# bioXiaoheng/BallerMixPlus

Measured on AMD Instinct MI355X. Metric: CLR windows/sec (B2 scan, n=100), higher is better.
Workload: dtype f64; 1 GPU; BASELINE config 4: synthetic whole genome, 39999999 SNPs over 22 chromosomes (GRCh37 proportions), n=100, default 31x10x51 (A,x,alpha) grid, B2 scan, every SNP a test site; site arrays of all chromosomes resident on every GPU, test sites dealt to the GPUs in blocks of 4096; grid_points=15810, library_build=8afc0fca11e6a83d

## Files before the change

### ballermixplus_amd/csrc/bmxscan.hip

```cpp
#include <hip/hip_runtime.h>
#include <stdint.h>
#include <stdio.h>
#include <stdlib.h>
#include <string.h>

#include <dlfcn.h>
#include <errno.h>
#include <rccl/rccl.h>

#include <algorithm>
#include <atomic>
#include <mutex>
#include <type_traits>
#include <string>
#include <thread>
#include <unordered_set>
#include <vector>

#include "../../include/bmxscan.h"
#include "bmx_math.h"

namespace {

thread_local std::string g_err;
// ... 1137 lines not shown
                    acc[i + 1] *= fma(Fs[i + 1], v0, 1.0);
                }
                __builtin_amdgcn_wave_barrier();
            } else {
                for (int b = L_int; b < R_int; b += SP) generic_pass(b, +1, R_int, staged);
            }
            PROF_MARK(0);
            int b = bulk_zone(R_int, +1, tL, t0);
            if (b != ZONE_DONE) { CNT(12, 1); while (!generic_pass(b, +1, N, false)) { b += SP; CNT(12, 1); } }
            PROF_MARK(7);
            b = bulk_zone(L_int - 1, -1, t0, tL);
            if (b != ZONE_DONE) { CNT(12, 1); while (!generic_pass(b, -1, -1, false)) { b -= SP; CNT(12, 1); } }
            PROF_MARK(7);

            renorm_all();
#pragma unroll
            for (int j = 0; j < J; ++j) {
                const int ec = min(max(E[j], -131071), 131071) + 131072;
                const int eb = bestK[j] >> 13;
                const bool better = (ec > eb) || (ec == eb && acc[j] > bestM[j]);
                if (better && p < P.npairs) {
                    bestM[j] = acc[j];
                    bestK[j] = (ec << 13) | iA;
                }
            }
        }
#pragma unroll
        for (int j = 0; j < J; ++j) {
            const int biA = bestK[j] & 8191;
            int bE = bestK[j] >> 13;
            double bM = bestM[j];
            int bL = biA == 8191 ? 0x7fffffff : biA * P.npairs + p;
            for (int off = 32; off > 0; off >>= 1) {
                const int oE = __shfl_xor(bE, off);
                const double oM = __shfl_xor(bM, off);
                const int oL = __shfl_xor(bL, off);
                if (oE > bE || (oE == bE && (oM > bM || (oM == bM && oL < bL)))) { bE = oE; bM = oM; bL = oL; }
            }
            if (lane == 0 && j < nvalid) {
                const size_t o = (size_t)slice * P.M + (tb + j);
                P.part_T[o] = bM;
                P.part_lin[o] = bL;
                P.part_ns[o] = bE;
            }
        }
    }
#ifdef BMX_PROFILE
    if (lane == 0 && P.prof)
        for (int k = 0; k < 12; ++k) atomicAdd(P.prof + k, (unsigned long long)prof_[k]);
#endif
#ifdef BMX_COUNT
    if (lane == 0 && P.prof)
        for (int k = 0; k < 16; ++k) atomicAdd(P.prof + 16 + k, cnt_[k]);
#endif
}

#ifndef BMX_P_ORDER
#define BMX_P_ORDER 12
#endif
constexpr int P_ORDER = BMX_P_ORDER;
constexpr int P_COPIES = 4;
static_assert(P_ORDER == 8 || P_ORDER == 12 || P_ORDER == 16, "far-field order of the prepared kernels: 8, 12 or 16");
static_assert(P_COPIES * P_ORDER <= WAVE, "slot-0 copies must fit one wave-wide read");
constexpr double P_EPS = P_ORDER == 16 ? 0.25 : P_ORDER == 12 ? 0.15 : 0.05;
constexpr int P_FAR_CAP = P_ORDER == 16 ? 2048 : P_ORDER == 12 ? 3584 : 8192;
#if BMX_P_ORDER == 16
__device__ constexpr double P_W[16] = {0.9999999999999954, 0.4999999999999791, 0.3333333333368442, 0.250000000008901, 0.19999999921757028,
                                       0.1666666652123534, 0.14285722101681053, 0.1250001188192722, 0.11110698172974029, 0.09999456222768308,
                                       0.09103227543438049, 0.08347880124963403, 0.07484961178075682, 0.06918273076087589, 0.08475562956871537,
                                       0.08074032343426385};
__device__ constexpr double P_D[14] = {9.539, 6.739, 5.071, 3.966, 3.181, 2.594, 2.14, 1.778, 1.483, 1.237, 1.03, 0.853, 0.7, 0.566};
#elif BMX_P_ORDER == 12
__device__ constexpr double P_W[12] = {0.9999999999999661, 0.49999999999988076, 0.3333333333754503, 0.25000000008463336, 0.19999998506452038,
                                       0.1666666441614055, 0.14285940976674, 0.1250028457483109, 0.11094429253027539, 0.09981580095968261,
                                       0.09676290425438011, 0.08920395582674094};
__device__ constexpr double P_D[10] = {9.029, 6.228, 4.56, 3.455, 2.67, 2.084, 1.629, 1.267, 0.972, 0.726};
#else
__device__ constexpr double P_W[8] = {0.9999999999998467, 0.4999999999996164, 0.3333333341509627, 0.25000000122701976,
                                      0.19999882322703955, 0.16666529319200146, 0.1434841013671569, 0.12562715480255862};
__device__ constexpr double P_D[6] = {7.94, 5.13, 3.462, 2.357, 1.571, 0.985};
#endif
constexpr double P_RAG_D = P_ORDER == 16 ? 6.74 : P_ORDER == 12 ? 6.23 : 5.13;
constexpr int PREP_HDR = 3, PREP_GUARD = 8, PREP_MOM = 1 + P_ORDER / 2, PREP_RAG_GUARD = 1;
constexpr double SER_DMIN = P_ORDER > 8 ? P_D[P_ORDER > 8 ? 6 : 0] : 0.0;
constexpr int SER_CAP = 64;
constexpr int PREP_MAGIC = 0x5a0e0000;
constexpr int RING_UNITS = 256, RING_MIRROR = 32, AUX_UNITS = 32;
constexpr int PREP_ZONE_DONE = -0x7fffffff;
constexpr int PREP_THREADS = 256;
constexpr int PREP_THR_LDS_MAX = 4096;
constexpr int64_t SOLO_GAP = 10;

struct PrepParams {
    const double *genpos;
    RowArray row;
    int64_t N;
    int rows, rowmul;
    const double *A;
    int nA;
    const double *test_gen;
    const int64_t *win_lo, *win_hi, *center, *center_hi;
    int64_t M;
    double zcut;
    const double *rowthr;
    int thr_in_lds;
    const uint8_t *kmom;
    const int *row_of_slot;
    int mom_slots;
    int ser_cap;
    int64_t g_begin, g_end;
    int32_t *blob_units;
    const int64_t *blob_prefix;
    int64_t prefix_base;
    ScratchEnt *arena;
    int *status;
};

template <int J, bool FILL>
__global__ __launch_bounds__(PREP_THREADS) void prep_kernel(PrepParams P) {
    extern __shared__ __attribute__((aligned(16))) double lds_p[];
    const int lane = threadIdx.x & (WAVE - 1);
    const int wave = __builtin_amdgcn_readfirstlane((int)(threadIdx.x >> 6));
    const int nw = blockDim.x / WAVE;
    const int N = (int)P.N;
    const int thr_len = P.thr_in_lds ? ((P.rows + 1) & ~1) : 0;
    if (P.thr_in_lds) {
        for (int idx = threadIdx.x; idx < P.rows; idx += blockDim.x) lds_p[idx] = P.rowthr[idx];
        __syncthreads();
    }
    constexpr int MS = FILL ? P_ORDER : 1;
    const int mom_len = (P.mom_slots + P_COPIES - 1 + 3) * MS;
    double *mom_r = lds_p + thr_len + wave * (2 * mom_len + WAVE);
    double *mom_l = mom_r + mom_len;
    double *ragscr = mom_l + mom_len;
    ScratchEnt *ser_r = reinterpret_cast<ScratchEnt *>(lds_p + thr_len + nw * (2 * mom_len + WAVE)) + wave * (2 * SER_CAP);
    ScratchEnt *ser_l = ser_r + SER_CAP;
    for (int idx = lane; idx < 2 * mom_len; idx += WAVE) mom_r[idx] = 0.0;
    __builtin_amdgcn_wave_barrier();
    const int64_t grp = P.g_begin + (int64_t)blockIdx.x * nw + wave;
    if (grp >= P.g_end) return;
    auto thr_of = [&](int r) -> double {
        double v;
        if (P.thr_in_lds) v = lds_p[r]; else v = P.rowthr[r];
        return v;
    };
    auto rank = [&](unsigned long long m) {
        return (int)__builtin_amdgcn_mbcnt_hi((unsigned)(m >> 32), __builtin_amdgcn_mbcnt_lo((unsigned)m, 0u));
    };
    constexpr int BS = J >= 16 ? 4 : 8;

    const int64_t tb = grp * J;
    const int nvalid = (int)min((int64_t)J, P.M - tb);
    const int jl = lane % J;
    const int jj = min(jl, nvalid - 1);
    const double tj = P.test_gen[tb + jj];
    int lo_j = (int)max(P.win_lo[tb + jj], (int64_t)0);
    int hi_j = (int)min(P.win_hi[tb + jj], (int64_t)N - 1);
    if (jl >= nvalid) { lo_j = 1; hi_j = 0; }
    const double t0 = readlane_f64(tj, 0), tL = readlane_f64(tj, J - 1);
    const int c0 = (int)P.center[tb], cU = (int)P.center_hi[tb + nvalid - 1];
    int lo_max = 0, hi_min = N - 1;
#pragma unroll
    for (int j = 0; j < J; ++j) {
        const int a = __builtin_amdgcn_readlane(lo_j, j), b = __builtin_amdgcn_readlane(hi_j, j);
        if (j < nvalid) { lo_max = max(lo_max, a); hi_min = min(hi_min, b); }
    }
    int L_int = min(c0, hi_min + 1), R_int = max(cU, lo_max);
    if (hi_min < lo_max) { L_int = c0; R_int = c0; hi_min = -1; lo_max = N; }

    int wpos = 0;
    ScratchEnt *out = nullptr;
    if (FILL) out = P.arena + (P.blob_prefix[grp] - P.prefix_base);

    for (int iA = 0; iA < P.nA; ++iA) {
        const double A = P.A[iA];
        const int kmom = min((int)P.kmom[iA], P.mom_slots);
        auto zone_near = [&](int base, int dir, double tnear, double tfar, double *mom, ScratchEnt *ser, int &zbase_o, int &npp_o, int &nqp_o,
                             int &nfar_o, int &base_o, double &m1p_o, double &m2p_o, int &nragv_o, int &nrmax_o, int &rag_o, double &zr_o,
                             int &rr_o, int &nser_o) {
            const int zbase = wpos, nbase = zbase + PREP_HDR;
            int n_pair = 0, n_pair_pad = 0, n_quad = 0, nfar_tot = 0, pad_ro = 0, n_ser = 0;
            bool pair_open = true, seen = false;
            double m1p = 0.0, m2p = 0.0;
            auto close_pairs = [&]() {
                n_pair_pad = (n_pair + BS - 1) & ~(BS - 1);
                if (FILL && lane < n_pair_pad - n_pair) out[nbase + n_pair + lane] = ScratchEnt{0.0, pad_ro, 0};
                pair_open = false;
            };
            int i = base + dir * lane;
            double g_nx = P.genpos[min(max(i, 0), N - 1)];
            int r_nx = (int)P.row[min(max(i, 0), N - 1)];
            while (true) {
                const bool ok = dir > 0 ? (i <= hi_min) : (i >= lo_max);
                const double g = g_nx;
                const int rraw = r_nx;
                const int inx = i + dir * WAVE;
                g_nx = P.genpos[min(max(inx, 0), N - 1)];
                r_nx = (int)P.row[min(max(inx, 0), N - 1)];
                const bool bulk = ok && (A * fabs(g - tfar) <= P.zcut);
                const int cnt = __popcll(__ballot(bulk));
                if (cnt) {
                    const double zn = A * fabs(g - tnear);
                    const double th = thr_of(rraw);
                    const int slot = __double2loint(th) & 0xff;
                    const bool farx = bulk && zn >= th && nfar_tot + n_ser < P_FAR_CAP;
                    const bool moml = farx && slot < kmom;
                    const bool serx = farx && slot >= kmom && !(zn - th < SER_DMIN);
                    const unsigned long long ms_ = __ballot(serx);
                    const bool ser_ok = n_ser + __popcll(ms_) <= P.ser_cap;
                    const bool serl = ser_ok && serx;
                    const bool nearl = bulk && !moml && !serl;
                    const bool pairl = nearl && zn < LN2;
                    const unsigned long long mm = __ballot(moml), mp = __ballot(pairl), mq = __ballot(nearl && !pairl);
                    const int nfar = __popcll(mm);
                    if (!seen) { pad_ro = __builtin_amdgcn_readlane(rraw, 0) * P.rowmul; seen = true; }
                    double Ev = 0.0;
                    if (FILL) Ev = bulk ? exp_neg(zn) : 0.0;
                    if (nfar) {
                        if (moml) {
                            double *mr = mom + (slot ? slot + P_COPIES - 1 : (lane & (P_COPIES - 1))) * MS;
                            if (FILL) {
                                const double d = zn - th;
                                const double E2 = Ev * Ev;
                                if (slot == 0) { m1p += Ev; m2p += E2; }
                                else { atomicAdd(mr, Ev); atomicAdd(mr + 1, E2); }
                                double Ek = E2;
#pragma unroll
                                for (int k = 3; k <= P_ORDER; ++k) {
                                    if (!(d < P_D[k - 3])) break;
                                    Ek *= Ev;
                                    atomicAdd(mr + (k - 1), Ek);
                                }
                            } else {
                                mom[(slot ? slot + P_COPIES - 1 : 0) * MS] = 1.0;
                            }
                        }
                        nfar_tot += nfar;
                    }
                    if (ser_ok && ms_ != 0ull) {
                        if (FILL && serl) {
                            const double d = zn - th;
                            const int cls = !(d < P_D[0]) ? 2 : !(d < P_D[1]) ? 3 : !(d < P_D[3]) ? 5 : 8;
                            ser[n_ser + rank(ms_)] = ScratchEnt{Ev, rraw * P.rowmul, cls};
                        }
                        n_ser += __popcll(ms_);
                    }
                    if (pair_open) {
                        if (FILL && pairl) out[nbase + n_pair + rank(mp)] = ScratchEnt{Ev, rraw * P.rowmul, 0};
                        n_pair += __popcll(mp);
                        if (__ballot(bulk && !(zn < LN2)) != 0ull || cnt < WAVE) close_pairs();
                    }
                    if (!pair_open) {
                        if (FILL && nearl && !pairl) out[nbase + n_pair_pad + n_quad + rank(mq)] = ScratchEnt{Ev, rraw * P.rowmul, 0};
                        n_quad += __popcll(mq);
                    }
                }
                base += dir * cnt;
                if (cnt < WAVE) break;
                i = inx;
            }
            if (pair_open) close_pairs();
            const int n_quad_pad = (n_quad + 3) & ~3;
            if (FILL) {
                if (lane < n_quad_pad - n_quad) out[nbase + n_pair_pad + n_quad + lane] = ScratchEnt{0.0, pad_ro, 0};
                if (lane < PREP_GUARD) out[nbase + n_pair_pad + n_quad_pad + lane] = ScratchEnt{0.0, pad_ro, 0};
            }
            wpos = nbase + n_pair_pad + n_quad_pad + PREP_GUARD;

            int nrag_v = 0, nrmax = 0;
            int rag = 0;
            double zr = 0.0;
            int rr = 0;
            {
                const int ir = base + dir * lane;
                const bool inr = ir >= 0 && ir < N;
                const int ic = min(max(ir, 0), N - 1);
                const double g = P.genpos[ic];
                rr = (int)P.row[ic];
                bool okr = __ballot(inr && (dir > 0 ? g <= tnear : g >= tnear)) == 0ull &&
                           __ballot(dir > 0 ? lo_j > base : hi_j < base) == 0ull;
                if (okr) {
                    ragscr[lane] = g;
                    __builtin_amdgcn_wave_barrier();
                    const int cnt1 = min(max(dir > 0 ? hi_j - base + 1 : base - lo_j + 1, 0), WAVE);
                    int lo_n = 0, hi_n = WAVE;
#pragma unroll
                    for (int it = 0; it < 7; ++it) {
                        const int mid = min((lo_n + hi_n) >> 1, WAVE - 1);
                        const bool pm = A * fabs(ragscr[mid] - tj) <= P.zcut;
                        const bool act = lo_n < hi_n;
                        lo_n = act && pm ? mid + 1 : lo_n;
                        hi_n = act && !pm ? mid : hi_n;
                    }
                    nrag_v = min(cnt1, lo_n);
                    __builtin_amdgcn_wave_barrier();
                    const int nb = dir > 0 ? __shfl_up(nrag_v, 1) : __shfl_down(nrag_v, 1);
                    const bool edge = dir > 0 ? jl == 0 : jl == J - 1;
                    okr = __ballot(!edge && nb > nrag_v) == 0ull;
                    nrmax = __builtin_amdgcn_readlane(nrag_v, dir > 0 ? J - 1 : 0);
                }
                if (okr && nrmax > 0 && nrmax < WAVE) {
                    zr = A * fabs(g - tnear);
                    const bool far8 = lane >= nrmax || zr >= thr_of(rr) + SER_DMIN;
                    const bool far3 = lane >= nrmax || zr >= thr_of(rr) + P_RAG_D;
                    rag = __ballot(far8) == ~0ull ? (__ballot(far3) == ~0ull ? 1 : 3) : 0;
                }
            }
            if (rag) {
                if (FILL) {
                    if (lane < nrmax) out[wpos + lane] = ScratchEnt{exp_neg(zr), rr * P.rowmul, zr >= thr_of(rr) + P_RAG_D ? 0 : 1};
                    if (lane == nrmax) out[wpos + lane] = ScratchEnt{0.0, rr * P.rowmul, 0};
                }
                wpos += nrmax + PREP_RAG_GUARD;
            }
            zbase_o = zbase; npp_o = n_pair_pad; nqp_o = n_quad_pad; nfar_o = nfar_tot; base_o = base; m1p_o = m1p; m2p_o = m2p;
            nragv_o = nrag_v; nrmax_o = nrmax; rag_o = rag; zr_o = zr; rr_o = rr; nser_o = n_ser;
        };
        auto zone_far = [&](double *mom, const ScratchEnt *ser, int n_ser, int zbase, int n_pair_pad, int n_quad_pad, int nfar_tot, int base,
                            double m1p, double m2p, int nrag_v, int nrmax, int rag, double zr, int rr) {
            int n_occ = 0;
            if (nfar_tot) {
                __builtin_amdgcn_wave_barrier();
                {
                    double x = 0.0;
                    if (lane < P_COPIES * MS) {
                        x = mom[lane];
                        mom[lane] = 0.0;
                    }
                    if (FILL) {
                        double y1 = m1p, y2 = m2p;
#pragma unroll
                        for (int off = 1; off < WAVE; off <<= 1) {
                            y1 += __shfl_xor(y1, off);
                            y2 += __shfl_xor(y2, off);
                        }
                        x += lane == 0 ? y1 : lane == 1 ? y2 : 0.0;
// ... 385 lines not shown
        int E[J], bestK[J];
#pragma unroll
        for (int j = 0; j < J; ++j) {
            bestM[j] = BMX_FREXP ? 0.5 : 1.0;
            bestK[j] = ((131072 + (BMX_FREXP ? 1 : 0)) << 13) | 8191;
        }

        for (int iA = 0; iA < P.nA; ++iA) {
            const double A = P.A[iA];
            int bits = 0;
#pragma unroll
            for (int j = 0; j < J; ++j) { acc[j] = 1.0; E[j] = 0; }
            auto renorm_all = [&]() {
#pragma unroll
                for (int j = 0; j < J; ++j) {
                    if (BMX_FREXP) renorm_fx(acc[j], E[j]); else renorm(acc[j], E[j]);
                }
                bits = 0;
            };
            auto spend = [&](int nbits) {
                if (bits + nbits > 1000) renorm_all();
                bits += nbits;
            };
            const int span_generic = max(P.span_hi, 54);

            auto apply_pass = [&](double alpha, int rowoff, unsigned long long m_in, double *buf) {
                buf[lane] = alpha;
                __builtin_amdgcn_wave_barrier();
                double Rpre[SP];
                if (!USE_LDS) {
#pragma unroll
                    for (int s = 0; s < SP; ++s) Rpre[s] = loadR(__builtin_amdgcn_readlane(rowoff, s * J));
                }
#pragma unroll
                for (int s = 0; s < SP; ++s) {
                    if (((m_in >> (s * J)) & ((1ull << J) - 1ull)) == 0ull) continue;
                    const double R = USE_LDS ? loadR(__builtin_amdgcn_readlane(rowoff, s * J)) : Rpre[s];
                    const double2 *a2 = reinterpret_cast<const double2 *>(buf + s * J);
#pragma unroll
                    for (int j = 0; j < J; j += 2) {
                        const double2 a = a2[j >> 1];
                        acc[j] *= fma(a.x, R, 1.0);
                        acc[j + 1] *= fma(a.y, R, 1.0);
                    }
                }
                __builtin_amdgcn_wave_barrier();
            };
            auto generic_core = [&](int i, bool inr, double g, int rowoff, int dir) -> bool {
                const bool inwin = inr && i >= lo_j && i <= hi_j;
                const double z = A * fabs(g - tj);
                const bool in = inwin && (z <= P.zcut) && (g != tj);
                const bool fin = lo_j > hi_j ||
                                 (dir > 0 ? (!inr || i > hi_j || (i >= lo_j && g > tj && z > P.zcut))
                                          : (!inr || i < lo_j || (i <= hi_j && g < tj && z > P.zcut)));
                const unsigned long long m_in = __ballot(in);
                if (m_in != 0ull) {
                    const double alpha = in ? exp_neg(z) : 0.0;
                    spend(SP * (__ballot(in && z < 0.6931471805599453) == 0ull ? max(P.span_hi, 2) : span_generic));
                    apply_pass(alpha, rowoff, m_in, scr_d);
                }
                return __ballot(fin) == ~0ull;
            };
            auto generic_pass = [&](int b, int dir, int lim, bool from_lds) -> bool {
                const int i = b + dir * sl;
                const bool inr = dir > 0 ? (i < lim) : (i > lim);
                double g = 0.0;
                int rowoff = 0;
                if (from_lds) {
                    if (inr) { g = mid_g[i - L_int]; rowoff = mid_ro[i - L_int]; }
                } else {
                    if (inr) { g = P.genpos[i]; rowoff = (int)P.row[i] * rowmul; }
                }
                return generic_core(i, inr, g, rowoff, dir);
            };

            auto zone_near = [&](auto dirk, double tnear, double &fv_o, int &nocc_o, int &nfar_o, int &nrmax_o, int &rag_o, int &nser_o,
                                 FargVec &farg) -> int {
                constexpr int dirc = decltype(dirk)::value;
                int nragv_o = 0;
                nocc_o = 0; nfar_o = 0; nrmax_o = 0; rag_o = 0; nser_o = 0;
                fv_o = 0.0;
                if (bad) return PREP_ZONE_DONE;
                double F[J];
                {
                    const double fv = exp_neg(A * fabs(tnear - tj));
                    fv_o = fv;
#pragma unroll
                    for (int j = 0; j < J; ++j) F[j] = readlane_f64(fv, j);
                }
                need();
                const int4 *hp = reinterpret_cast<const int4 *>(ring + (pos & (RING_UNITS - 1)));
                const int4 h0 = hp[0], h1 = hp[1];
                const int magic = __builtin_amdgcn_readfirstlane(h0.x);
                const int n_pair = __builtin_amdgcn_readfirstlane(h0.y), n_quad = __builtin_amdgcn_readfirstlane(h0.z);
                const int n_occ = __builtin_amdgcn_readfirstlane(h0.w);
                const int nfar_tot = __builtin_amdgcn_readfirstlane(h1.x), nrmax = __builtin_amdgcn_readfirstlane(h1.y);
                const int base_end = __builtin_amdgcn_readfirstlane(h1.z), ser_w = __builtin_amdgcn_readfirstlane(h1.w);
                const int n_ser = ser_w & 0xff, c8 = (ser_w >> 8) & 0xff, c5 = (ser_w >> 16) & 0xff, c3 = (ser_w >> 24) & 0xff;
                const int rag = magic & 3;
                if ((magic & ~3) != PREP_MAGIC || rag == 2 || n_pair < 0 || n_quad < 0 || n_pair > N + 8 || n_quad > N + 8 || n_occ < 0 || n_occ > MOM_SLOTS ||
                    nrmax < 0 || nrmax >= WAVE || n_ser > SER_CAP || (n_ser & 3) || c8 > c5 || c5 > c3 || c3 > n_ser) {
                    bad = true;
                    return PREP_ZONE_DONE;
                }
                nragv_o = (int)reinterpret_cast<const unsigned char *>(hp + 2)[jl];
                nocc_o = n_occ; nfar_o = nfar_tot; nrmax_o = nrmax; rag_o = rag; nser_o = ser_w;
                pos += PREP_HDR;
                PROF_MARK(1);

                if (n_pair > 0) {
                    need();
                    const double e0 = ring[pos & (RING_UNITS - 1)].e;
                    const double om = 1.0 - e0, op = fma(e0, P.rmax, 1.0);
                    const int pend_lo = 1024 - ((__builtin_amdgcn_readfirstlane(__double2hiint(om)) >> 20) & 0x7ff);
                    const int pend_hi = ((__builtin_amdgcn_readfirstlane(__double2hiint(op)) >> 20) & 0x7ff) - 1022;
                    const int span8 = 8 * min(max(pend_hi, pend_lo), 125);
                    double Rp[BS], ep[BS];
                    if (BMX_PPAIR_PREFETCH) {
                        const ScratchEnt *rp = ring + (pos & (RING_UNITS - 1));
#pragma unroll
                        for (int u = 0; u < BS; ++u) {
                            const ScratchEnt en = rp[u];
                            ep[u] = en.e;
                            Rp[u] = loadR(en.ro);
                        }
                    }
                    for (int l0 = 0; l0 < n_pair; l0 += BS) {
                        need();
                        const ScratchEnt *rp = ring + (pos & (RING_UNITS - 1));
                        spend(span8 * BS / 8);
                        double v[BS];
                        if (BMX_PPAIR_PREFETCH) {
#pragma unroll
                            for (int u = 0; u < BS; ++u) v[u] = ep[u] * Rp[u];
#pragma unroll
                            for (int u = 0; u < BS; ++u) {
                                const ScratchEnt en = rp[BS + u];
                                ep[u] = en.e;
                                Rp[u] = loadR(en.ro);
                            }
                        } else {
#pragma unroll
                            for (int u = 0; u < BS; ++u) {
                                const ScratchEnt en = rp[u];
                                v[u] = en.e * loadR(en.ro);
                            }
                        }
#pragma unroll
                        for (int u = 0; u < BS; u += 2) {
                            const double sv = v[u] + v[u + 1], qv = v[u] * v[u + 1];
#pragma unroll
                            for (int j = 0; j < J; ++j) acc[j] *= fma(F[j], fma(F[j], qv, sv), 1.0);
                        }
                        pos += BS;
                    }
                }
                PROF_MARK(2);
                if (n_quad > 0) {
                    need();
                    int span8q = 0;
                    double Rn[4], en_e[4];
                    {
                        const ScratchEnt *rp = ring + (pos & (RING_UNITS - 1));
#pragma unroll
                        for (int u = 0; u < 4; ++u) {
                            const ScratchEnt en = rp[u];
                            en_e[u] = en.e;
                            Rn[u] = loadR(en.ro);
                        }
                    }
                    for (int l0 = 0; l0 < n_quad; l0 += 4) {
                        need();
                        const ScratchEnt *rp = ring + (pos & (RING_UNITS - 1));
                        if ((l0 & 63) == 0) {
                            const double op = fma(rp[0].e, P.rmax, 1.0);
                            const int hi = ((__builtin_amdgcn_readfirstlane(__double2hiint(op)) >> 20) & 0x7ff) - 1022;
                            span8q = 8 * min(max(hi, 2), 125);
                        }
                        spend(span8q / 2);
                        double v[4];
#pragma unroll
                        for (int u = 0; u < 4; ++u) v[u] = en_e[u] * Rn[u];
#pragma unroll
                        for (int u = 0; u < 4; ++u) {
                            const ScratchEnt en = rp[4 + u];
                            en_e[u] = en.e;
                            Rn[u] = loadR(en.ro);
                        }
                        const double s01 = v[0] + v[1], q01 = v[0] * v[1];
                        const double s23 = v[2] + v[3], q23 = v[2] * v[3];
                        const double e1 = s01 + s23;
                        const double e2 = fma(s01, s23, q01 + q23);
                        const double e3 = fma(q01, s23, q23 * s01);
                        const double e4 = q01 * q23;
#pragma unroll
                        for (int j = 0; j < J; ++j) {
                            double t = fma(F[j], e4, e3);
                            t = fma(F[j], t, e2);
                            t = fma(F[j], t, e1);
                            acc[j] *= fma(F[j], t, 1.0);
                            if ((j & (BMX_QSB - 1)) == BMX_QSB - 1) __builtin_amdgcn_sched_barrier(0);
                        }
                        pos += 4;
                    }
                }
                PROF_MARK(3);
                pos += PREP_GUARD;
                if (rag) {
                    need();
                    const bool rag_hi = (rag & 2) != 0;
                    const ScratchEnt ragm = ring[(pos + lane) & (RING_UNITS - 1)];
                    double rag_R0 = loadR(__builtin_amdgcn_readlane(ragm.ro, 0));
                    double rag_R1 = loadR(__builtin_amdgcn_readlane(ragm.ro, min(1, nrmax)));
                    double rag_R2 = loadR(__builtin_amdgcn_readlane(ragm.ro, min(2, nrmax)));
                    const int nrag_v = nragv_o;
                    double r1 = 0.0, r2 = 0.0, r3 = 0.0;
                    int l = 0, ph = 0;
                    if (USE_LDS) {
#pragma unroll
                        for (int w = 0; w < J; ++w) {
                            const int j = dirc > 0 ? w : J - 1 - w;
                            rag_walk_lds(l, __builtin_amdgcn_readlane(nrag_v, j), nrmax, __double2loint(ragm.e), __double2hiint(ragm.e), ragm.ro,
                                         lds_lane_addr, rag_R0, rag_R1, rag_R2, r1, r2, r3);
                            const double f = F[j];
                            farg[j] = fma(-f, fma(-f, fma(-f, r3, r2), r1), farg[j]);
                        }
                        rag_walk_settle(rag_R0, rag_R1, rag_R2);
                    } else {
#pragma unroll
                        for (int w = 0; w < J; ++w) {
                            const int j = dirc > 0 ? w : J - 1 - w;
                            rag_walk_global(l, ph, __builtin_amdgcn_readlane(nrag_v, j), nrmax, __double2loint(ragm.e), __double2hiint(ragm.e), ragm.ro,
                                            lane8, Rb, rag_R0, rag_R1, rag_R2, r1, r2, r3);
                            const double f = F[j];
                            farg[j] = fma(-f, fma(-f, fma(-f, r3, r2), r1), farg[j]);
                        }
                        rag_walk_settle_global(rag_R0, rag_R1, rag_R2);
                    }
                    if (rag_hi) {
                        for (int lh = 0; lh < nrmax; ++lh) {
                            if (__builtin_amdgcn_readlane(ragm.pad, lh) == 0) continue;
                            const double v = readlane_f64(ragm.e, lh) * loadR(__builtin_amdgcn_readlane(ragm.ro, lh));
#pragma unroll
                            for (int j = 0; j < J; ++j) {
                                const double u = (lh < __builtin_amdgcn_readlane(nrag_v, j)) ? F[j] * v : 0.0;
                                const double u2 = u * u;
                                double t = fma(-u, P_W[7], P_W[6]);
                                t = fma(-u, t, P_W[5]);
                                t = fma(-u, t, P_W[4]);
                                t = fma(-u, t, P_W[3]);
                                farg[j] = fma(u2 * u2, t, farg[j]);
                            }
                        }
                    }
                    pos += nrmax + PREP_RAG_GUARD;
                }
                PROF_MARK(7);
                return base_end;
            };

            auto zone_far = [&](double fv, int n_occ, int ser_w, int nfar_tot, FargVec &farg) {
                const int n_ser = ser_w & 0xff, ser_cls = ser_w >> 8;
                if (bad || !nfar_tot) return;
                double F[J];
#pragma unroll
                for (int j = 0; j < J; ++j) F[j] = readlane_f64(fv, j);
                double pk[P_ORDER];
#pragma unroll
                for (int k = 0; k < P_ORDER; ++k) pk[k] = 0.0;
                auto fold = [&](const double m1, const double2 *q, const double R) {
                    double pw[P_ORDER + 1];
                    pw[1] = R;
#pragma unroll
                    for (int k = 2; k <= P_ORDER; ++k) pw[k] = pw[k >> 1] * pw[k - (k >> 1)];
                    pk[0] = fma(m1, R, pk[0]);
#pragma unroll
                    for (int k = 2; k <= P_ORDER; ++k) {
                        const double2 v = q[(k - 2) >> 1];
                        pk[k - 1] = fma((k & 1) ? v.y : v.x, pw[k], pk[k - 1]);
                    }
                };
                if (BMX_FOLD_EARLY && n_occ > 0) {
                    need();
                    const ScratchEnt *rp0 = ring + (pos & (RING_UNITS - 1));
                    ScratchEnt ua = rp0[0], ub = rp0[n_occ > 1 ? PREP_MOM : 0];
                    double Ra = loadR(ua.ro), Rb2 = loadR(ub.ro);
                    for (int s = 0; s < n_occ; s += 2) {
                        need();
                        const ScratchEnt *rp = ring + (pos & (RING_UNITS - 1));
                        const bool two = s + 1 < n_occ;
                        const double m1a = ua.e, m1b = ub.e, Rca = Ra, Rcb = Rb2;
                        const int na = s + 2 < n_occ ? 2 * PREP_MOM : 0, nb = s + 3 < n_occ ? 3 * PREP_MOM : na;
                        ua = rp[na];
                        ub = rp[nb];
                        Ra = loadR(ua.ro);
                        Rb2 = loadR(ub.ro);
                        fold(m1a, reinterpret_cast<const double2 *>(rp + 1), Rca);
                        if (two) fold(m1b, reinterpret_cast<const double2 *>(rp + PREP_MOM + 1), Rcb);
                        pos += two ? 2 * PREP_MOM : PREP_MOM;
                    }
                }
                if (!BMX_FOLD_EARLY) {
                    for (int s = 0; s < n_occ; s += 2) {
                        need();
                        const ScratchEnt *rp = ring + (pos & (RING_UNITS - 1));
                        const bool two = s + 1 < n_occ;
                        const ScratchEnt ua = rp[0], ub = rp[two ? PREP_MOM : 0];
                        const double Ra = loadR(ua.ro), Rb2 = loadR(ub.ro);
                        fold(ua.e, reinterpret_cast<const double2 *>(rp + 1), Ra);
                        if (two) fold(ub.e, reinterpret_cast<const double2 *>(rp + PREP_MOM + 1), Rb2);
                        pos += two ? 2 * PREP_MOM : PREP_MOM;
                    }
                }
                PROF_MARK(5);
                if (n_ser > 0) {
                    need();
                    const ScratchEnt mine = ring[(pos + lane) & (RING_UNITS - 1)];
                    const int e8 = (ser_cls & 0x7f) + 3 & ~3, e5 = max(e8, ((ser_cls >> 8) & 0x7f) + 3 & ~3), e3 = max(e5, ((ser_cls >> 16) & 0x7f) + 3 & ~3);
                    double Rn[4];
#pragma unroll
                    for (int u = 0; u < 4; ++u) Rn[u] = loadR(__builtin_amdgcn_readlane(mine.ro, u));
                    auto batch = [&](auto kc, int s0) {
                        constexpr int K = decltype(kc)::value;
                        double Rc[4];
#pragma unroll
                        for (int u = 0; u < 4; ++u) Rc[u] = Rn[u];
                        const int nx = s0 + 4 < n_ser ? s0 + 4 : s0;
#pragma unroll
                        for (int u = 0; u < 4; ++u) Rn[u] = loadR(__builtin_amdgcn_readlane(mine.ro, nx + u));
#pragma unroll
                        for (int u = 0; u < 4; ++u) {
                            const double v = readlane_f64(mine.e, s0 + u) * Rc[u];
                            pk[0] += v;
                            if (K == 2) {
                                pk[1] = fma(v, v, pk[1]);
                            } else {
                                const double v2 = v * v;
                                pk[1] += v2;
                                pk[2] = fma(v2, v, pk[2]);
                                if (K > 3) {
                                    const double v4 = v2 * v2;
                                    pk[3] += v4;
                                    pk[4] = fma(v4, v, pk[4]);
                                    if (K > 5) {
                                        pk[5] = fma(v4, v2, pk[5]);
                                        pk[6] = fma(v4 * v2, v, pk[6]);
                                        pk[7] = fma(v4, v4, pk[7]);
                                    }
                                }
                            }
                        }
                    };
                    int s0 = 0;
                    for (; s0 < e8; s0 += 4) batch(std::integral_constant<int, 8>{}, s0);
                    for (; s0 < e5; s0 += 4) batch(std::integral_constant<int, 5>{}, s0);
                    for (; s0 < e3; s0 += 4) batch(std::integral_constant<int, 3>{}, s0);
                    for (; s0 < n_ser; s0 += 4) batch(std::integral_constant<int, 2>{}, s0);
                    pos += n_ser;
                }
                PROF_MARK(6);
#pragma unroll
                for (int k = 0; k < P_ORDER; ++k) pk[k] *= P_W[k];
#pragma unroll
                for (int j = 0; j < J; ++j) {
                    const double f = F[j];
                    double t = pk[P_ORDER - 1];
#pragma unroll
                    for (int k = P_ORDER - 2; k >= 0; --k) t = fma(-f, t, pk[k]);
                    farg[j] = fma(-f, t, farg[j]);
                }
                PROF_MARK(7);
            };

            PROF_MARK(9);
            if (BMX_MIDTRI && mid_tri && A * (tL - t0) <= P.zcut) {
                const double xk = A * (tj - t0);
                double Gk, Hk;
                exp_neg2(xk, -xk, Gk, Hk);
                const int ro_k = mid_ro[jl];
                spend((J - 1) * span_generic);
                double Fs[J];
#pragma unroll
                for (int j = 0; j < J; ++j) Fs[j] = readlane_f64(Hk, j);
                if (lane < J) scr[lane] = ScratchEnt{Gk, ro_k, 0};
                __builtin_amdgcn_wave_barrier();
#pragma unroll
                for (int i = 0; i < J; i += 2) {
                    const ScratchEnt en0 = scr[i], en1 = scr[i + 1];
                    const double v1 = en1.e * loadR(en1.ro);
                    if (i > 0) {
                        const double v0 = en0.e * loadR(en0.ro);
                        const double sv = v0 + v1, qv = v0 * v1;
#pragma unroll
                        for (int j = 0; j < i; ++j) acc[j] *= fma(Fs[j], fma(Fs[j], qv, sv), 1.0);
                    }
                    acc[i] *= fma(Fs[i], v1, 1.0);
                }
                __builtin_amdgcn_wave_barrier();
#pragma unroll
                for (int j = 0; j < J; ++j) Fs[j] = readlane_f64(Gk, j);
                if (lane < J) scr[lane] = ScratchEnt{Hk, ro_k, 0};
                __builtin_amdgcn_wave_barrier();
#pragma unroll
                for (int i = 0; i < J; i += 2) {
                    const ScratchEnt en0 = scr[i], en1 = scr[i + 1];
                    const double v0 = en0.e * loadR(en0.ro);
                    if (i + 2 < J) {
                        const double v1 = en1.e * loadR(en1.ro);
                        const double sv = v0 + v1, qv = v0 * v1;
#pragma unroll
                        for (int j = i + 2; j < J; ++j) acc[j] *= fma(Fs[j], fma(Fs[j], qv, sv), 1.0);
                    }
                    acc[i + 1] *= fma(Fs[i + 1], v0, 1.0);
                }
                __builtin_amdgcn_wave_barrier();
            } else {
                for (int b = L_int; b < R_int; b += SP) generic_pass(b, +1, R_int, staged);
            }
            PROF_MARK(0);
            double fvR, fvL;
            int noccR, nfarR, nrmR, nserR, noccL, nfarL, nrmL, nserL;
            int ragR, ragL;
            FargVec farg;
#pragma unroll
            for (int j = 0; j < J; ++j) farg[j] = 0.0;
            int b = zone_near(std::integral_constant<int, +1>{}, tL, fvR, noccR, nfarR, nrmR, ragR, nserR, farg);
            if (b != PREP_ZONE_DONE) { while (!generic_pass(b, +1, N, false)) b += SP; }
            PROF_MARK(4);
            b = zone_near(std::integral_constant<int, -1>{}, t0, fvL, noccL, nfarL, nrmL, ragL, nserL, farg);
            if (b != PREP_ZONE_DONE) { while (!generic_pass(b, -1, -1, false)) b -= SP; }
            PROF_MARK(4);
            if (!bad && (nfarR || ragR || nfarL || ragL)) {
                auto apply_far = [&]() {
#pragma unroll
                    for (int w = 0; w < J; w += 2) {
                        double e0, e1;
                        exp_neg2(farg[w], farg[w + 1], e0, e1);
                        acc[w] *= e0;
                        acc[w + 1] *= e1;
                        asm volatile("" : "+v"(acc[w]), "+v"(acc[w + 1]));
                        farg[w] = 0.0;
                        farg[w + 1] = 0.0;
                    }
                    PROF_MARK(8);
                };
                const int bitsR = 2 + (int)((float)(nfarR + nrmR) * P.far_bits), bitsL = 2 + (int)((float)(nfarL + nrmL) * P.far_bits);
                const bool split = bitsR + bitsL > 900;
                zone_far(fvR, noccR, nserR, nfarR, farg);
                if (split) {
                    spend(bitsR);
                    apply_far();
                }
                zone_far(fvL, noccL, nserL, nfarL, farg);
                spend(split ? bitsL : bitsR + bitsL);
                apply_far();
            }

            renorm_all();
#pragma unroll
            for (int j = 0; j < J; ++j) {
                const int ec = min(max(E[j], -131071), 131071) + 131072;
// ... 2675 lines not shown
    if (J == 8) fn = GPICK(8);
    else if (J == 16) fn = GPICK(16);
    else if (J == 4) fn = GPICK(4);
    else if (solo) fn = PICK(clr_scan_solo_kernel);
    else fn = PICK(clr_scan_kernel);
#define GPL(JJ) (use_lds ? (const void *)clr_scan_prepared_kernel<JJ, true, true> : (const void *)clr_scan_prepared_kernel<JJ, false, true>)
    const void *fn_pl = nullptr;
    if (mode == 4 && J == 16) fn_pl = GPL(16);
    else if (mode == 4 && J == 8) fn_pl = GPL(8);
    else if (mode == 4 && J == 4) fn_pl = GPL(4);
    else if (solo) fn_pl = use_lds ? (const void *)clr_scan_solo_kernel<true, true> : (const void *)clr_scan_solo_kernel<false, true>;
#undef GPL
#undef GP2
#undef GP4
#undef GPICK
#undef PICK
    int threads = SCAN_THREADS;
    size_t lds_bytes = (use_lds ? lds + (J ? lds_rm : 0) : 0) + (J ? (size_t)(threads / WAVE) * wave_bytes(mom_slots) : 0);
    if (J && 2 * lds_bytes > (size_t)LDS_LIMIT_BYTES) {
        threads = SCAN_THREADS_MAX;
        lds_bytes = (use_lds ? lds + lds_rm : 0) + (size_t)(threads / WAVE) * wave_bytes(mom_slots);
        spb *= 2;
    }
    if (prepared && J == 8 && use_lds) {
        const size_t lds12 = lds + (size_t)(SCAN_THREADS_J8 / WAVE) * wave_bytes(mom_slots);
        if (lds12 <= (size_t)LDS_LIMIT_BYTES) {
            if (threads == SCAN_THREADS_MAX) spb /= 2;
            threads = SCAN_THREADS_J8;
            lds_bytes = lds12;
            spb = spb * 3;
        }
    }
    if (!J) {
        threads = SITE_THREADS;
        lds_bytes = (use_lds ? lds : 0) + (size_t)(threads / WAVE) * (solo ? wave_bytes(0) : SITE_SCR * sizeof(ScratchEnt));
    }
    if (lds_bytes > (size_t)LDS_LIMIT_BYTES) return fail(BMX_E_LIMIT, "LDS budget exceeded");
    if (lds_bytes) HIP_TRY(hipFuncSetAttribute(fn, hipFuncAttributeMaxDynamicSharedMemorySize, (int)lds_bytes));
    P.sites_per_block = spb;
    pl.fn = fn; pl.fn_pl = fn_pl; pl.J = solo ? 1 : J; pl.threads = threads; pl.lds_bytes = lds_bytes; pl.spb = spb; pl.use_lds = use_lds;
    pl.mode = solo ? 5 : J ? mode : -1;
    int64_t range = std::max<int64_t>((int64_t)(512u << 20) / (16 * (int64_t)c->nslices), spb);
    range = std::min<int64_t>(range, (int64_t)0x7fffff00LL / c->nslices * spb);
    if (const int64_t plb = pl_bytes_per_test(c, c->pl_which)) range = std::min<int64_t>(range, std::max<int64_t>(PL_SCRATCH_BYTES / plb, spb));
    range = std::max<int64_t>(range / spb, 1) * spb;
    pl.range = range;
    if (prepared || solo) {
        pl.thr_in_lds = c->rows <= PREP_THR_LDS_MAX ? 1 : 0;
        const int pm = std::max(1, std::min(use_lds ? MOM_SLOTS_LDS : MOM_SLOTS, (prepared && J == 16) ? s->kmom_max_ser : s->kmom_max));
        P.mom_slots = pm;
        const size_t mom_fill = solo ? (size_t)(pm + S_COPIES - 1 + 3) * S_ORDER : 2 * (size_t)(pm + P_COPIES - 1 + 3) * P_ORDER + WAVE;
        const size_t mom_count = solo ? mom_fill : 2 * (size_t)(pm + P_COPIES - 1 + 3) + WAVE;
        pl.prep_threads = mom_fill * sizeof(double) > 20480 ? PREP_THREADS / 4 : PREP_THREADS;
        const size_t thr_b = pl.thr_in_lds ? (size_t)((c->rows + 1) & ~1) * sizeof(double) : 0;
        const size_t stage_b = solo ? (size_t)(SOLO_S0 + 2 * SOLO_S1) * sizeof(double) : 2 * SER_CAP * sizeof(ScratchEnt);
        pl.prep_lds = thr_b + (size_t)(pl.prep_threads / WAVE) * (mom_fill * sizeof(double) + stage_b);
        pl.prep_lds_count = thr_b + (size_t)(pl.prep_threads / WAVE) * (mom_count * sizeof(double) + (solo ? stage_b : 0));
        P.far_bits = (float)(P_EPS * 1.4427 * 1.1);
        if (P_ORDER == 16) P.far_bits = (float)(P_EPS * 1.4427 * 1.2);
#define PP(JJ, FF) (const void *)prep_kernel<JJ, FF>
        if (solo) {
            pl.prep_count = (const void *)prep_solo_kernel<false>;
            pl.prep_fill = (const void *)prep_solo_kernel<true>;
        } else {
            pl.prep_count = J == 16 ? PP(16, false) : J == 8 ? PP(8, false) : PP(4, false);
            pl.prep_fill = J == 16 ? PP(16, true) : J == 8 ? PP(8, true) : PP(4, true);
        }
#undef PP
        if (pl.prep_lds > (size_t)LDS_LIMIT_BYTES) return fail(BMX_E_LIMIT, "LDS budget of the preparation kernel exceeded");
        HIP_TRY(hipFuncSetAttribute(pl.prep_count, hipFuncAttributeMaxDynamicSharedMemorySize, (int)pl.prep_lds_count));
        HIP_TRY(hipFuncSetAttribute(pl.prep_fill, hipFuncAttributeMaxDynamicSharedMemorySize, (int)pl.prep_lds));
    }
    TRACE("scan plan: lds=%zu use_lds=%d span_hi=%d spb=%d J=%d threads=%d range=%lld mode=%d", lds_bytes, (int)use_lds, c->span_hi, spb, J, threads,
          (long long)range, pl.mode);
    return BMX_OK;
}

PrepParams prep_params(bmx_ctx *c, ChromSlot *s, const ScanPlan &pl) {
    PrepParams Q;
    Q.genpos = s->genpos.p; Q.row = pl.P.row; Q.N = s->N;
    Q.rows = c->rows; Q.rowmul = pl.use_lds ? WAVE : c->NP;
    Q.A = c->d_A; Q.nA = c->nA;
    Q.test_gen = s->test_gen.p; Q.win_lo = s->win_lo.p; Q.win_hi = s->win_hi.p; Q.center = s->center.p; Q.center_hi = s->center_hi.p;
    Q.M = s->M; Q.zcut = c->zcut;
    Q.rowthr = s->rowthr.p; Q.thr_in_lds = pl.thr_in_lds;
    const bool series = pl.mode == 4 && pl.J == 16;
    Q.kmom = s->kmom.p + (series ? c->nA : 0); Q.row_of_slot = s->d_row_of_slot.p; Q.mom_slots = pl.P.mom_slots;
    Q.ser_cap = !series ? 0 : diag_env("BMX_SER_CAP") ? std::min(std::max(atoi(diag_env("BMX_SER_CAP")), 0), SER_CAP) : SER_CAP;
    Q.g_begin = 0; Q.g_end = 0;
    Q.blob_units = s->blob_units.p; Q.blob_prefix = s->blob_prefix.p; Q.prefix_base = 0;
    Q.arena = c->arena.p; Q.status = c->d_status;
    return Q;
}

int ensure_prep(bmx_ctx *c, ChromSlot *s) {
    ScanPlan &pl = s->plan;
    if (pl.mode < 4 || s->prep_ok) return BMX_OK;
    const int J = pl.J;
    const int64_t ngroups = (s->M + J - 1) / J;
    HIP_TRY(s->blob_units.ensure((size_t)ngroups));
    HIP_TRY(s->blob_prefix.ensure((size_t)ngroups + 1));
    PrepParams Q = prep_params(c, s, pl);
    Q.g_begin = 0; Q.g_end = ngroups;
    const int gpw = pl.prep_threads / WAVE;
    void *kargs[] = {&Q};
    {
        std::lock_guard<std::mutex> launch_lock(g_launch_mu);
        if (pl.prep_lds_count) HIP_TRY(hipFuncSetAttribute(pl.prep_count, hipFuncAttributeMaxDynamicSharedMemorySize, (int)pl.prep_lds_count));
        HIP_TRY(hipLaunchKernel(pl.prep_count, dim3((unsigned)((ngroups + gpw - 1) / gpw)), dim3(pl.prep_threads), kargs, pl.prep_lds_count, c->stream));
    }
    hipLaunchKernelGGL(prefix_kernel, dim3(1), dim3(1024), 0, c->stream, (const int32_t *)s->blob_units.p, ngroups, s->blob_prefix.p);
    HIP_TRY(hipGetLastError());
    std::vector<int64_t> pre((size_t)ngroups + 1);
    HIP_TRY(hipMemcpyAsync(pre.data(), s->blob_prefix.p, pre.size() * sizeof(int64_t), hipMemcpyDeviceToHost, c->stream));
    HIP_TRY(hipStreamSynchronize(c->stream));
    size_t free_b = 0, total_b = 0;
    HIP_TRY(hipMemGetInfo(&free_b, &total_b));
    const int64_t cap_units = (int64_t)(std::min<size_t>((free_b + c->arena.cap * sizeof(ScratchEnt)) / 4, (size_t)16 << 30) / sizeof(ScratchEnt));
    const int64_t gstep = std::max<int64_t>(pl.spb / J, 1);
    s->ranges.clear();
    int64_t need = 0;
    for (int64_t g0 = 0; g0 < ngroups;) {
        int64_t g1 = g0;
        while (g1 < ngroups) {
            const int64_t g2 = std::min(g1 + gstep, ngroups);
            if (g1 > g0 && ((g2 - g0) * J > pl.range || pre[(size_t)g2] - pre[(size_t)g0] > cap_units)) break;
            g1 = g2;
        }
        const int64_t units = pre[(size_t)g1] - pre[(size_t)g0];
        if (units > cap_units) return fail(BMX_E_LIMIT, "prepared scan: one workgroup's share of the stream does not fit the device memory left");
        s->ranges.push_back(PrepRange{g0 * J, std::min(g1 * J, s->M) - g0 * J, g0, g1 - g0, pre[(size_t)g0], units});
        need = std::max(need, units);
        g0 = g1;
    }
    const size_t want = (size_t)need + 8 * WAVE;
    HIP_TRY(c->arena.ensure(s->has_orig && want > c->arena.cap ? want + want / 8 : want));
    TRACE("prepared: %lld groups, %.1f MB of blobs, %zu launch range(s), arena %.1f MB", (long long)ngroups, (double)pre[(size_t)ngroups] * 16e-6,
          s->ranges.size(), (double)c->arena.cap * 16e-6);
    s->prep_ok = true;
    return BMX_OK;
}

int ensure_plan(bmx_ctx *c, ChromSlot *s) {
    if (!s->plan_ok || s->plan_variant != c->variant || s->plan_pl != c->pl_which) {
        s->plan_ok = false;
        s->prep_ok = false;
        int rc = plan_scan(c, s, s->plan);
        if (rc) return rc;
        s->plan_ok = true;
        s->plan_variant = c->variant;
        s->plan_pl = c->pl_which;
    }
    return ensure_prep(c, s);
}

int launch_range(bmx_ctx *c, ChromSlot *s, ScanPlan &pl, int64_t off, int64_t cnt, const PrepRange *pr) {
    std::lock_guard<std::mutex> launch_lock(g_launch_mu);
    ScanParams P = pl.P;
    const size_t np = (size_t)cnt * c->nslices;
    HIP_TRY(c->part_T.ensure(np));
    HIP_TRY(c->part_lin.ensure(np));
    HIP_TRY(c->part_ns.ensure(np));
    P.test_gen = s->test_gen.p + off; P.win_lo = s->win_lo.p + off; P.win_hi = s->win_hi.p + off;
    P.center = s->center.p + off; P.center_hi = s->center_hi.p + off; P.M = cnt;
    P.part_T = c->part_T.p; P.part_lin = c->part_lin.p; P.part_ns = c->part_ns.p;
    const int plw = c->pl_which;
    const void *fn = plw ? pl.fn_pl : pl.fn;
// ... 1548 lines not shown
```

Measured before the change: 4.783 million windows/s.

## Precompute per-zone exponentials and span codes in prep kernel stream

Moves the per-A mid-triangle exponentials (G,H), each zone's near factor exp(-A|tnear-tj|), and the pair/quad span codes from the scan kernel into the preparation kernel. These are written into the scratch stream as extra headers and pad fields. The scan kernel then reads them from the ring instead of recomputing exponentials and exponent-bit spans per group and A. It also restructures the series batch loop so an optional two-register-set ping-pong (off by default) can be enabled. The trade is a larger stream and more ring traffic in exchange for fewer transcendental evaluations and less serial scalar work in the hot kernel.

Result: no change. 4.805 million windows/s, median of 6 (+0.5%).

```diff
diff --git a/ballermixplus_amd/csrc/bmxscan.hip b/ballermixplus_amd/csrc/bmxscan.hip
--- a/ballermixplus_amd/csrc/bmxscan.hip
+++ b/ballermixplus_amd/csrc/bmxscan.hip
@@ -1243,6 +1243,25 @@
 #endif
 constexpr double P_RAG_D = P_ORDER == 16 ? 6.74 : P_ORDER == 12 ? 6.23 : 5.13;
 constexpr int PREP_HDR = 3, PREP_GUARD = 8, PREP_MOM = 1 + P_ORDER / 2, PREP_RAG_GUARD = 1;
+#ifndef BMX_UNIFORM_STREAM
+#define BMX_UNIFORM_STREAM 1
+#endif
+#ifndef BMX_SER_TWOSETS
+#define BMX_SER_TWOSETS 0
+#endif
+constexpr int prep_fhdr(int J) { return BMX_UNIFORM_STREAM ? J / 2 : 0; }
+constexpr int prep_ahdr(int J) { return BMX_UNIFORM_STREAM ? J : 0; }
+__device__ __forceinline__ int near_span_pair(double e0, double rmax) {
+    const double om = 1.0 - e0, op = fma(e0, rmax, 1.0);
+    const int pend_lo = 1024 - ((__double2hiint(om) >> 20) & 0x7ff);
+    const int pend_hi = ((__double2hiint(op) >> 20) & 0x7ff) - 1022;
+    return 8 * min(max(pend_hi, pend_lo), 125);
+}
+__device__ __forceinline__ int near_span_quad(double e0, double rmax) {
+    const double op = fma(e0, rmax, 1.0);
+    const int hi = ((__double2hiint(op) >> 20) & 0x7ff) - 1022;
+    return 8 * min(max(hi, 2), 125);
+}
 constexpr double SER_DMIN = P_ORDER > 8 ? P_D[P_ORDER > 8 ? 6 : 0] : 0.0;
 constexpr int SER_CAP = 64;
 constexpr int PREP_MAGIC = 0x5a0e0000;
@@ -1263,6 +1282,7 @@
     const int64_t *win_lo, *win_hi, *center, *center_hi;
     int64_t M;
     double zcut;
+    double rmax;
     const double *rowthr;
     int thr_in_lds;
     const uint8_t *kmom;
@@ -1336,13 +1356,29 @@
     for (int iA = 0; iA < P.nA; ++iA) {
         const double A = P.A[iA];
         const int kmom = min((int)P.kmom[iA], P.mom_slots);
+        if (BMX_UNIFORM_STREAM) {
+            if (FILL) {
+                double Gk = 0.0, Hk = 0.0;
+                if (A * (tL - t0) <= P.zcut) {
+                    const double xk = A * (tj - t0);
+                    exp_neg2(xk, -xk, Gk, Hk);
+                }
+                if (lane < J) {
+                    double *o = reinterpret_cast<double *>(out + wpos);
+                    o[lane] = Gk;
+                    o[J + lane] = Hk;
+                }
+            }
+            wpos += prep_ahdr(J);
+        }
         auto zone_near = [&](int base, int dir, double tnear, double tfar, double *mom, ScratchEnt *ser, int &zbase_o, int &npp_o, int &nqp_o,
                              int &nfar_o, int &base_o, double &m1p_o, double &m2p_o, int &nragv_o, int &nrmax_o, int &rag_o, double &zr_o,
                              int &rr_o, int &nser_o) {
-            const int zbase = wpos, nbase = zbase + PREP_HDR;
+            const int zbase = wpos, nbase = zbase + PREP_HDR + prep_fhdr(J);
             int n_pair = 0, n_pair_pad = 0, n_quad = 0, nfar_tot = 0, pad_ro = 0, n_ser = 0;
             bool pair_open = true, seen = false;
             double m1p = 0.0, m2p = 0.0;
+            if (BMX_UNIFORM_STREAM && FILL && lane < J) reinterpret_cast<double *>(out + zbase + PREP_HDR)[lane] = exp_neg(A * fabs(tnear - tj));
             auto close_pairs = [&]() {
                 n_pair_pad = (n_pair + BS - 1) & ~(BS - 1);
                 if (FILL && lane < n_pair_pad - n_pair) out[nbase + n_pair + lane] = ScratchEnt{0.0, pad_ro, 0};
@@ -1407,12 +1443,12 @@
                         n_ser += __popcll(ms_);
                     }
                     if (pair_open) {
-                        if (FILL && pairl) out[nbase + n_pair + rank(mp)] = ScratchEnt{Ev, rraw * P.rowmul, 0};
+                        if (FILL && pairl) out[nbase + n_pair + rank(mp)] = ScratchEnt{Ev, rraw * P.rowmul, BMX_UNIFORM_STREAM ? near_span_pair(Ev, P.rmax) : 0};
                         n_pair += __popcll(mp);
                         if (__ballot(bulk && !(zn < LN2)) != 0ull || cnt < WAVE) close_pairs();
                     }
                     if (!pair_open) {
-                        if (FILL && nearl && !pairl) out[nbase + n_pair_pad + n_quad + rank(mq)] = ScratchEnt{Ev, rraw * P.rowmul, 0};
+                        if (FILL && nearl && !pairl) out[nbase + n_pair_pad + n_quad + rank(mq)] = ScratchEnt{Ev, rraw * P.rowmul, BMX_UNIFORM_STREAM ? near_span_quad(Ev, P.rmax) : 0};
                         n_quad += __popcll(mq);
                     }
                 }
@@ -1964,7 +2000,7 @@
                 fv_o = 0.0;
                 if (bad) return PREP_ZONE_DONE;
                 double F[J];
-                {
+                if (!BMX_UNIFORM_STREAM) {
                     const double fv = exp_neg(A * fabs(tnear - tj));
                     fv_o = fv;
 #pragma unroll
@@ -1972,6 +2008,12 @@
                 }
                 need();
                 const int4 *hp = reinterpret_cast<const int4 *>(ring + (pos & (RING_UNITS - 1)));
+                if (BMX_UNIFORM_STREAM) {
+                    const double fv = reinterpret_cast<const double *>(hp + PREP_HDR)[jl];
+                    fv_o = fv;
+#pragma unroll
+                    for (int j = 0; j < J; ++j) F[j] = readlane_f64(fv, j);
+                }
                 const int4 h0 = hp[0], h1 = hp[1];
                 const int magic = __builtin_amdgcn_readfirstlane(h0.x);
                 const int n_pair = __builtin_amdgcn_readfirstlane(h0.y), n_quad = __builtin_amdgcn_readfirstlane(h0.z);
@@ -1987,16 +2029,21 @@
                 }
                 nragv_o = (int)reinterpret_cast<const unsigned char *>(hp + 2)[jl];
                 nocc_o = n_occ; nfar_o = nfar_tot; nrmax_o = nrmax; rag_o = rag; nser_o = ser_w;
-                pos += PREP_HDR;
+                pos += PREP_HDR + prep_fhdr(J);
                 PROF_MARK(1);
 
                 if (n_pair > 0) {
                     need();
-                    const double e0 = ring[pos & (RING_UNITS - 1)].e;
-                    const double om = 1.0 - e0, op = fma(e0, P.rmax, 1.0);
-                    const int pend_lo = 1024 - ((__builtin_amdgcn_readfirstlane(__double2hiint(om)) >> 20) & 0x7ff);
-                    const int pend_hi = ((__builtin_amdgcn_readfirstlane(__double2hiint(op)) >> 20) & 0x7ff) - 1022;
-                    const int span8 = 8 * min(max(pend_hi, pend_lo), 125);
+                    int span8;
+                    if (BMX_UNIFORM_STREAM) {
+                        span8 = __builtin_amdgcn_readfirstlane(ring[pos & (RING_UNITS - 1)].pad);
+                    } else {
+                        const double e0 = ring[pos & (RING_UNITS - 1)].e;
+                        const double om = 1.0 - e0, op = fma(e0, P.rmax, 1.0);
+                        const int pend_lo = 1024 - ((__builtin_amdgcn_readfirstlane(__double2hiint(om)) >> 20) & 0x7ff);
+                        const int pend_hi = ((__builtin_amdgcn_readfirstlane(__double2hiint(op)) >> 20) & 0x7ff) - 1022;
+                        span8 = 8 * min(max(pend_hi, pend_lo), 125);
+                    }
                     double Rp[BS], ep[BS];
                     if (BMX_PPAIR_PREFETCH) {
                         const ScratchEnt *rp = ring + (pos & (RING_UNITS - 1));
@@ -2055,9 +2102,13 @@
                         need();
                         const ScratchEnt *rp = ring + (pos & (RING_UNITS - 1));
                         if ((l0 & 63) == 0) {
-                            const double op = fma(rp[0].e, P.rmax, 1.0);
-                            const int hi = ((__builtin_amdgcn_readfirstlane(__double2hiint(op)) >> 20) & 0x7ff) - 1022;
-                            span8q = 8 * min(max(hi, 2), 125);
+                            if (BMX_UNIFORM_STREAM) {
+                                span8q = __builtin_amdgcn_readfirstlane(rp[0].pad);
+                            } else {
+                                const double op = fma(rp[0].e, P.rmax, 1.0);
+                                const int hi = ((__builtin_amdgcn_readfirstlane(__double2hiint(op)) >> 20) & 0x7ff) - 1022;
+                                span8q = 8 * min(max(hi, 2), 125);
+                            }
                         }
                         spend(span8q / 2);
                         double v[4];
@@ -2199,17 +2250,14 @@
                     need();
                     const ScratchEnt mine = ring[(pos + lane) & (RING_UNITS - 1)];
                     const int e8 = (ser_cls & 0x7f) + 3 & ~3, e5 = max(e8, ((ser_cls >> 8) & 0x7f) + 3 & ~3), e3 = max(e5, ((ser_cls >> 16) & 0x7f) + 3 & ~3);
-                    double Rn[4];
+                    double Rn[4], Rm[4];
 #pragma unroll
                     for (int u = 0; u < 4; ++u) Rn[u] = loadR(__builtin_amdgcn_readlane(mine.ro, u));
-                    auto batch = [&](auto kc, int s0) {
+                    auto batch2 = [&](auto kc, int s0, double (&Rc)[4], double (&Rx)[4]) {
                         constexpr int K = decltype(kc)::value;
-                        double Rc[4];
-#pragma unroll
-                        for (int u = 0; u < 4; ++u) Rc[u] = Rn[u];
                         const int nx = s0 + 4 < n_ser ? s0 + 4 : s0;
 #pragma unroll
-                        for (int u = 0; u < 4; ++u) Rn[u] = loadR(__builtin_amdgcn_readlane(mine.ro, nx + u));
+                        for (int u = 0; u < 4; ++u) Rx[u] = loadR(__builtin_amdgcn_readlane(mine.ro, nx + u));
 #pragma unroll
                         for (int u = 0; u < 4; ++u) {
                             const double v = readlane_f64(mine.e, s0 + u) * Rc[u];
@@ -2234,10 +2282,23 @@
                         }
                     };
                     int s0 = 0;
-                    for (; s0 < e8; s0 += 4) batch(std::integral_constant<int, 8>{}, s0);
-                    for (; s0 < e5; s0 += 4) batch(std::integral_constant<int, 5>{}, s0);
-                    for (; s0 < e3; s0 += 4) batch(std::integral_constant<int, 3>{}, s0);
-                    for (; s0 < n_ser; s0 += 4) batch(std::integral_constant<int, 2>{}, s0);
+                    auto run = [&](auto kc, int end) {
+                        if (BMX_SER_TWOSETS) {
+                            for (; s0 + 4 < end; s0 += 8) {
+                                batch2(kc, s0, Rn, Rm);
+                                batch2(kc, s0 + 4, Rm, Rn);
+                            }
+                        }
+                        for (; s0 < end; s0 += 4) {
+                            batch2(kc, s0, Rn, Rm);
+#pragma unroll
+                            for (int u = 0; u < 4; ++u) Rn[u] = Rm[u];
+                        }
+                    };
+                    run(std::integral_constant<int, 8>{}, e8);
+                    run(std::integral_constant<int, 5>{}, e5);
+                    run(std::integral_constant<int, 3>{}, e3);
+                    run(std::integral_constant<int, 2>{}, n_ser);
                     pos += n_ser;
                 }
                 PROF_MARK(6);
@@ -2255,10 +2316,21 @@
             };
 
             PROF_MARK(9);
+            const double *gh = nullptr;
+            if (BMX_UNIFORM_STREAM) {
+                need();
+                gh = reinterpret_cast<const double *>(ring + (pos & (RING_UNITS - 1)));
+                pos += prep_ahdr(J);
+            }
             if (BMX_MIDTRI && mid_tri && A * (tL - t0) <= P.zcut) {
-                const double xk = A * (tj - t0);
                 double Gk, Hk;
-                exp_neg2(xk, -xk, Gk, Hk);
+                if (BMX_UNIFORM_STREAM) {
+                    Gk = gh[jl];
+                    Hk = gh[J + jl];
+                } else {
+                    const double xk = A * (tj - t0);
+                    exp_neg2(xk, -xk, Gk, Hk);
+                }
                 const int ro_k = mid_ro[jl];
                 spend((J - 1) * span_generic);
                 double Fs[J];
@@ -5100,7 +5172,7 @@
     Q.rows = c->rows; Q.rowmul = pl.use_lds ? WAVE : c->NP;
     Q.A = c->d_A; Q.nA = c->nA;
     Q.test_gen = s->test_gen.p; Q.win_lo = s->win_lo.p; Q.win_hi = s->win_hi.p; Q.center = s->center.p; Q.center_hi = s->center_hi.p;
-    Q.M = s->M; Q.zcut = c->zcut;
+    Q.M = s->M; Q.zcut = c->zcut; Q.rmax = c->rmax;
     Q.rowthr = s->rowthr.p; Q.thr_in_lds = pl.thr_in_lds;
     const bool series = pl.mode == 4 && pl.J == 16;
     Q.kmom = s->kmom.p + (series ? c->nA : 0); Q.row_of_slot = s->d_row_of_slot.p; Q.mom_slots = pl.P.mom_slots;
```
